# GabeTsai/YOLO-For-Turbines

Measured on AMD Instinct MI355X. Metric: images/sec at 416x416 (fwd), higher is better.
Workload: dtype f32; 1 GPU; BASELINE configs[1]: batch 32/GPU 416x416 fp32 inference, 80-class head, YOLOv3 forward (75 fused conv launches); per_gpu_batch=32, global_batch=32, image_size=416, num_classes=80, parallelism=image-sharded x1 (no collective)

## Files before the change

yolo_for_turbines_amd/csrc/conv_wino4s_f32.hip:

```cpp
#include "split3.h"
#include "wino4_planes.h"
#include "wino4_epilogue.h"

namespace yolo {

struct Wino4SArgs {
    Wino4Args e;
    int nkc;
    int xmap;
};

constexpr int W4S_STAGE = 2 * W4S_PIECE;
constexpr int W4S_SLOTS = 4;
constexpr int W4S_DMA = 3;

template <int OFF>
__device__ __forceinline__ void w4s_read_at(s3_u32x4& f, unsigned addr) {
    asm volatile("ds_read_b128 %0, %1 offset:%2" : "=&v"(f) : "v"(addr), "n"(OFF));
}

template <int ACT, bool RES>
__global__ __launch_bounds__(512, 1) void conv_wino4s_f32(const Wino4SArgs q) {
    extern __shared__ __attribute__((aligned(16))) char smem[];
    const Wino4Args& p = q.e;
    const int tid = threadIdx.x, lane = tid & 63;
    const int wave = __builtin_amdgcn_readfirstlane(tid >> 6);
    const int l16 = lane & 15, kq = lane >> 4;
    const int xcd = blockIdx.x & 7, bq = blockIdx.x >> 3;
    const int row = bq / p.n_nt, wrows = (p.n_whole + 7) >> 3;
    int nt = bq % p.n_nt;
    bool cut = row >= wrows;
    int half = (row - wrows) & 1;
    int mt = cut ? p.n_whole + ((row - wrows) >> 1) * 8 + xcd : row * 8 + xcd;
    if (q.xmap) {
        const int sb = xcd + 8 * (bq >> 5), l = bq & 31, ntg = p.n_mt >> 2;
        cut = true;
        half = l & 1;
        nt = 4 * (sb / ntg) + ((l >> 1) & 3);
        mt = 4 * (sb % ntg) + (l >> 3);
    }
    if (mt >= (cut ? p.n_mt : p.n_whole)) return;
    const int wm = cut ? half : wave & 1, wn = cut ? wave & 3 : wave >> 1;
    const bool busy = !cut || wave < 4;

    int* tab = reinterpret_cast<int*>(smem + W4S_SLOTS * W4S_STAGE);
    wino4_tile_table(p, tab, tid, mt, cut, half);

    const bool dv = cut ? wave >= 4 : wave < 4;
    const int dw = cut ? (wave + 4) & 7 : wave;
    const unsigned own = cut && dv ? (wave - 4) * W4S_PLANE + half * (W4S_PLANE / 2) : 3072 * dw;
    const char* src = (dv ? reinterpret_cast<const char*>(p.V) + (size_t)mt * W4S_PIECE : reinterpret_cast<const char*>(p.U) + (size_t)nt * W4S_PIECE)
                      + (own - (dv ? 0 : W4S_PIECE));
    const size_t s_st = (size_t)(dv ? p.n_mt : p.n_nt) * W4S_PIECE;
    const unsigned lane16 = lane * 16;
    const unsigned lds0 = (unsigned)(size_t)(wn_lptr)smem;
    const unsigned ldsw = lds0 + own;
    const int nkc = q.nkc;
    auto issue_piece = [&](int k, int pass, int g, int slot) {
        const int kc = g / 6, x = g - 6 * kc;
        wn_glds16_s(src + ((size_t)(6 * pass + x) * nkc + kc) * s_st + k * 1024, lane16, ldsw + slot * W4S_STAGE + k * 1024);
    };
    auto issue = [&](int pass, int g, int slot) { wn_for<0, W4S_DMA>([&](auto K) { issue_piece(decltype(K)::value, pass, g, slot); }); };

    const unsigned sw = w4s_slot(l16, kq) * 16;
    const unsigned vb = lds0 + (32 * wm + l16) * 64 + sw;
    const unsigned ub = lds0 + W4S_PIECE + (16 * wn + l16) * 64 + sw;

    f32x4 py[2][4][4];
#pragma unroll
    for (int bb = 0; bb < 2; ++bb)
#pragma unroll
        for (int i = 0; i < 4; ++i)
#pragma unroll
            for (int j = 0; j < 4; ++j) py[bb][i][j] = f32x4{0.f, 0.f, 0.f, 0.f};

    auto run_pass = [&](auto PASS) {
        constexpr int a = decltype(PASS)::value;
        s3_u32x4 uh[2], vh[2][2], um, ul, vm[2], vl[2];
        auto rd_hi = [&](auto SET, unsigned sb) {
            constexpr int S = decltype(SET)::value;
            w4s_read_at<0>(uh[S], ub + sb);
            w4s_read_at<0>(vh[S][0], vb + sb);
            w4s_read_at<1024>(vh[S][1], vb + sb);
        };
        auto rd_vlo = [&](unsigned sb) {
            w4s_read_at<2 * W4S_PLANE>(vl[0], vb + sb);
            w4s_read_at<2 * W4S_PLANE + 1024>(vl[1], vb + sb);
        };
        auto rd_ulo = [&](unsigned sb) { w4s_read_at<2 * W4S_PLANE>(ul, ub + sb); };
        auto rd_vmid = [&](unsigned sb) {
            w4s_read_at<W4S_PLANE>(vm[0], vb + sb);
            w4s_read_at<W4S_PLANE + 1024>(vm[1], vb + sb);
        };
        auto rd_umid = [&](unsigned sb) { w4s_read_at<W4S_PLANE>(um, ub + sb); };
        auto mma = [&](f32x4 (&c)[2], const s3_u32x4& u, const s3_u32x4 (&v)[2]) {
            const s3_bf16x8 fa = __builtin_bit_cast(s3_bf16x8, u);
            c[0] = __builtin_amdgcn_mfma_f32_16x16x32_bf16(fa, __builtin_bit_cast(s3_bf16x8, v[0]), c[0], 0, 0, 0);
            c[1] = __builtin_amdgcn_mfma_f32_16x16x32_bf16(fa, __builtin_bit_cast(s3_bf16x8, v[1]), c[1], 0, 0, 0);
        };
        if constexpr (a == 0) {
            issue(0, 0, 0);
            issue(0, 1, 1);
            issue(0, 2, 2);
        }
        __builtin_amdgcn_sched_barrier(0);
        f32x4 acc[6][2];
#pragma unroll
        for (int x = 0; x < 6; ++x)
#pragma unroll
            for (int bb = 0; bb < 2; ++bb) acc[x][bb] = f32x4{0.f, 0.f, 0.f, 0.f};
#pragma unroll
        for (int x = 0; x < 6; ++x) asm volatile("" : "+v"(acc[x][0]), "+v"(acc[x][1]));
        __builtin_amdgcn_sched_barrier(0);
        wn_wait_vmcnt<2 * W4S_DMA>();
        __builtin_amdgcn_s_barrier();
        __builtin_amdgcn_sched_barrier(0);
        rd_hi(std::integral_constant<int, 0>{}, 0u);
        rd_vlo(0u);
        rd_ulo(0u);
        rd_vmid(0u);
        rd_umid(0u);

        for (int kc = 0; kc < nkc; ++kc) {
            const bool more = kc + 1 < nkc;
            wn_for<0, 6>([&](auto X) {
                constexpr int x = decltype(X)::value, set = x & 1;
                const int g = 6 * kc + x;
                const bool next = x < 5 || more;
                const bool ahead = x < 3 || more;
                const unsigned nb = (unsigned)((g + 1) & (W4S_SLOTS - 1)) * W4S_STAGE;
                const int as = (g + 3) & (W4S_SLOTS - 1);
                __builtin_amdgcn_sched_barrier(0);
                if (next) {
                    if (x < 4 || more) wn_wait_vmcnt<W4S_DMA>();
                    else wn_wait_vmcnt<0>();
                    __builtin_amdgcn_s_barrier();
                }
                __builtin_amdgcn_sched_barrier(0);
                rd_hi(std::integral_constant<int, set ^ 1>{}, nb);
                asm volatile("s_waitcnt lgkmcnt(7)" : "+v"(uh[set]), "+v"(vl[0]), "+v"(vl[1]));
                mma(acc[x], uh[set], vl);
                __builtin_amdgcn_sched_barrier(0);
                if (ahead) issue_piece(0, a, g + 3, as);
                rd_vlo(nb);
                asm volatile("s_waitcnt lgkmcnt(8)" : "+v"(ul), "+v"(vh[set][0]), "+v"(vh[set][1]));
                __builtin_amdgcn_sched_barrier(0);
                mma(acc[x], ul, vh[set]);
                __builtin_amdgcn_sched_barrier(0);
                if (ahead) issue_piece(1, a, g + 3, as);
                rd_ulo(nb);
                asm volatile("s_waitcnt lgkmcnt(6)" : "+v"(um), "+v"(vm[0]), "+v"(vm[1]));
                __builtin_amdgcn_sched_barrier(0);
                mma(acc[x], um, vm);
                __builtin_amdgcn_sched_barrier(0);
                if (ahead) issue_piece(2, a, g + 3, as);
                __builtin_amdgcn_sched_barrier(0);
                mma(acc[x], uh[set], vm);
                __builtin_amdgcn_sched_barrier(0);
                rd_vmid(nb);
                __builtin_amdgcn_sched_barrier(0);
                mma(acc[x], um, vh[set]);
                __builtin_amdgcn_sched_barrier(0);
                rd_umid(nb);
                __builtin_amdgcn_sched_barrier(0);
                mma(acc[x], uh[set], vh[set]);
            });
        }
        asm volatile("s_waitcnt lgkmcnt(0)" ::: "memory");
        __syncthreads();
        if constexpr (a < 5) {
            issue(a + 1, 0, 0);
            issue(a + 1, 1, 1);
            issue(a + 1, 2, 2);
            __builtin_amdgcn_sched_barrier(0);
        }
        wino4_fold_row<a>(acc, py);
    };
    if (busy) {
        run_pass(std::integral_constant<int, 0>{});
        run_pass(std::integral_constant<int, 1>{});
        run_pass(std::integral_constant<int, 2>{});
        run_pass(std::integral_constant<int, 3>{});
        run_pass(std::integral_constant<int, 4>{});
        run_pass(std::integral_constant<int, 5>{});
    } else {
        constexpr int HD = 2;
        const bool mover = wave < 7;
        auto issue_half = [&](int pass, int g, int slot) {
            if (mover) {
                issue_piece(0, pass, g, slot);
                issue_piece(1, pass, g, slot);
            }
        };
        const int ng = 6 * nkc;
        for (int a = 0; a < 6; ++a) {
            if (a == 0) {
                issue_half(0, 0, 0);
                issue_half(0, 1, 1);
                issue_half(0, 2, 2);
            }
            wn_wait_vmcnt<2 * HD>();
            __builtin_amdgcn_s_barrier();
            for (int g = 0; g < ng; ++g) {
                if (g + 1 < ng) {
                    if (g + 2 < ng) wn_wait_vmcnt<HD>();
                    else wn_wait_vmcnt<0>();
                    __builtin_amdgcn_s_barrier();
                }
                if (g + 3 < ng) issue_half(a, g + 3, (g + 3) & (W4S_SLOTS - 1));
            }
            __syncthreads();
            if (a < 5) {
                issue_half(a + 1, 0, 0);
                issue_half(a + 1, 1, 1);
                issue_half(a + 1, 2, 2);
            }
        }
    }

    wino4_epilogue<ACT, RES>(p, smem, tab, py, tid, nt, wm, wn, l16, kq, busy);
}

bool wino4_split_eligible(const yolo_conv_desc* d) {
    if (!wino4_split_supported(d) || d->h != d->w) return false;
    if (d->h == 26 && d->cin == 256 && d->cout == 512) return true;
    if ((d->h == 13 || d->h == 19) && d->cin == 512 && d->cout == 1024) return true;
    return d->h == 52 && d->cin == 128 && d->cout == 256;
}

int conv_wino4s_launch(const yolo_conv_desc* d, const void* x, const float* U4, const void* U_planes, const float* scale, const float* shift,
                       const void* residual, void* y, void* workspace, size_t workspace_bytes, int32_t* nan_flag, hipStream_t s) {
    const Wino4Geom g = wino4_geom(d);
    if (!g.planes) return fail(YOLO_ERR_UNSUPPORTED, "conv winograd F(4x4) on bf16 planes: needs fp32 3x3 stride 1, NHWC output, cin %% 32 == 0");
    const size_t need = g.v_plane_bytes + g.u_plane_bytes;
    if (!workspace || workspace_bytes < need) return fail(YOLO_ERR_WORKSPACE, "conv winograd F(4x4) on bf16 planes: workspace %zu < %zu bytes", workspace_bytes, need);
    if ((size_t)workspace & 15) return fail(YOLO_ERR_ARG, "conv winograd F(4x4) on bf16 planes: workspace must be 16-byte aligned");
    if (!U4 || ((size_t)U4 & 15)) return fail(YOLO_ERR_ARG, "conv winograd F(4x4) on bf16 planes: transformed filters must be 16-byte aligned");
    if ((size_t)U_planes & 15) return fail(YOLO_ERR_ARG, "conv winograd F(4x4) on bf16 planes: filter planes must be 16-byte aligned");
    if (int rc = wino4_planes_launch(g, d, x, U4, U_planes, workspace, s)) return rc;

    Wino4SArgs q;
    Wino4Args& a = q.e;
    a = wino4_gemm_args(g, d, scale, shift, residual, y, nan_flag);
    a.V = (const float*)workspace;
    a.U = (const float*)wino4_u_planes(g, U_planes, workspace);
    q.nkc = g.nkc;
    q.xmap = a.n_whole == 0 && a.n_mt % 4 == 0 && a.n_nt % 4 == 0 && (a.n_mt / 4) * (a.n_nt / 4) % 8 == 0;
    const int grid = q.xmap ? 2 * a.n_mt * a.n_nt : wino4_grid(a);
    const bool res = d->flags & YOLO_FLAG_RESIDUAL;
    const size_t lds = (size_t)W4S_SLOTS * W4S_STAGE + W4_TAB;
    auto go = [&](auto kern) -> int {
        static LdsOnce once;
        if (int rc = reserve_lds(once, reinterpret_cast<const void*>(kern), lds, "conv_wino4s_f32")) return rc;
        hipLaunchKernelGGL(kern, dim3(grid), dim3(512), lds, s, q);
        return check_launch("conv_wino4s_f32");
    };
    YOLO_SWITCH_ACT(d->act, return res ? go(&conv_wino4s_f32<ACT, true>) : go(&conv_wino4s_f32<ACT, false>));
    return fail(YOLO_ERR_ARG, "conv winograd F(4x4) on bf16 planes: activation");
}

}
```

Baseline: 3083 images/s.

## Deepen Winograd split-kernel LDS pipeline to six slots and prefetch across passes

Raises the LDS ring from four to six stage slots so the global-to-LDS loads run five stages ahead instead of three, with each stage's slot fixed by its Winograd index. The prefetch now runs continuously across the six passes, so the next pass's first stages are issued during the tail of the current one. This removes the per-pass __syncthreads and drain/refill bubble. It needs more LDS, which may limit occupancy or the shapes that fit. Per-stage vmcnt waits are rewritten by hand for the final lap, and the epilogue recomputes lane ids with mbcnt.

```diff
diff --git a/yolo_for_turbines_amd/csrc/conv_wino4s_f32.hip b/yolo_for_turbines_amd/csrc/conv_wino4s_f32.hip
--- a/yolo_for_turbines_amd/csrc/conv_wino4s_f32.hip
+++ b/yolo_for_turbines_amd/csrc/conv_wino4s_f32.hip
@@ -11,8 +11,10 @@
 };
 
 constexpr int W4S_STAGE = 2 * W4S_PIECE;
-constexpr int W4S_SLOTS = 4;
+constexpr int W4S_SLOTS = 6;
+constexpr int W4S_AHEAD = W4S_SLOTS - 1;
 constexpr int W4S_DMA = 3;
+static_assert(W4S_SLOTS == 6 && W4S_AHEAD == 5, "the slot of a stage is its xi, and the counted waits of the last lap are written out for five stages ahead");
 
 template <int OFF>
 __device__ __forceinline__ void w4s_read_at(s3_u32x4& f, unsigned addr) {
@@ -56,11 +58,10 @@
     const unsigned lds0 = (unsigned)(size_t)(wn_lptr)smem;
     const unsigned ldsw = lds0 + own;
     const int nkc = q.nkc;
-    auto issue_piece = [&](int k, int pass, int g, int slot) {
-        const int kc = g / 6, x = g - 6 * kc;
-        wn_glds16_s(src + ((size_t)(6 * pass + x) * nkc + kc) * s_st + k * 1024, lane16, ldsw + slot * W4S_STAGE + k * 1024);
+    auto issue_piece = [&](int k, int pass, int kc, int x) {
+        const int xi = kc < nkc ? 6 * pass + x : 6 * pass + 6 + x, c = kc < nkc ? kc : 0;
+        wn_glds16_s(src + ((size_t)xi * nkc + c) * s_st + k * 1024, lane16, ldsw + x * W4S_STAGE + k * 1024);
     };
-    auto issue = [&](int pass, int g, int slot) { wn_for<0, W4S_DMA>([&](auto K) { issue_piece(decltype(K)::value, pass, g, slot); }); };
 
     const unsigned sw = w4s_slot(l16, kq) * 16;
     const unsigned vb = lds0 + (32 * wm + l16) * 64 + sw;
@@ -99,9 +100,7 @@
             c[1] = __builtin_amdgcn_mfma_f32_16x16x32_bf16(fa, __builtin_bit_cast(s3_bf16x8, v[1]), c[1], 0, 0, 0);
         };
         if constexpr (a == 0) {
-            issue(0, 0, 0);
-            issue(0, 1, 1);
-            issue(0, 2, 2);
+            wn_for<0, W4S_AHEAD>([&](auto X) { wn_for<0, W4S_DMA>([&](auto K) { issue_piece(decltype(K)::value, 0, 0, decltype(X)::value); }); });
         }
         __builtin_amdgcn_sched_barrier(0);
         f32x4 acc[6][2];
@@ -112,8 +111,10 @@
 #pragma unroll
         for (int x = 0; x < 6; ++x) asm volatile("" : "+v"(acc[x][0]), "+v"(acc[x][1]));
         __builtin_amdgcn_sched_barrier(0);
-        wn_wait_vmcnt<2 * W4S_DMA>();
-        __builtin_amdgcn_s_barrier();
+        if constexpr (a == 0) {
+            wn_wait_vmcnt<(W4S_AHEAD - 1) * W4S_DMA>();
+            __builtin_amdgcn_s_barrier();
+        }
         __builtin_amdgcn_sched_barrier(0);
         rd_hi(std::integral_constant<int, 0>{}, 0u);
         rd_vlo(0u);
@@ -125,15 +126,18 @@
             const bool more = kc + 1 < nkc;
             wn_for<0, 6>([&](auto X) {
                 constexpr int x = decltype(X)::value, set = x & 1;
-                const int g = 6 * kc + x;
-                const bool next = x < 5 || more;
-                const bool ahead = x < 3 || more;
-                const unsigned nb = (unsigned)((g + 1) & (W4S_SLOTS - 1)) * W4S_STAGE;
-                const int as = (g + 3) & (W4S_SLOTS - 1);
+                const bool on = a < 5 || more;
+                const bool next = x < 5 || on;
+                const bool ahead = x < 1 || on;
+                constexpr int ax = (x + W4S_AHEAD) % W4S_SLOTS;
+                const int akc = x < 1 ? kc : kc + 1;
+                unsigned nb = (unsigned)((x + 1) % W4S_SLOTS) * W4S_STAGE;
+                asm volatile("" : "+s"(nb));
                 __builtin_amdgcn_sched_barrier(0);
                 if (next) {
-                    if (x < 4 || more) wn_wait_vmcnt<W4S_DMA>();
-                    else wn_wait_vmcnt<0>();
+                    constexpr int young = x < 2 ? W4S_AHEAD - 2 : x < 4 ? 4 - x : 0;
+                    if (on) wn_wait_vmcnt<(W4S_AHEAD - 2) * W4S_DMA>();
+                    else wn_wait_vmcnt<young * W4S_DMA>();
                     __builtin_amdgcn_s_barrier();
                 }
                 __builtin_amdgcn_sched_barrier(0);
@@ -141,19 +145,19 @@
                 asm volatile("s_waitcnt lgkmcnt(7)" : "+v"(uh[set]), "+v"(vl[0]), "+v"(vl[1]));
                 mma(acc[x], uh[set], vl);
                 __builtin_amdgcn_sched_barrier(0);
-                if (ahead) issue_piece(0, a, g + 3, as);
+                if (ahead) issue_piece(0, a, akc, ax);
                 rd_vlo(nb);
                 asm volatile("s_waitcnt lgkmcnt(8)" : "+v"(ul), "+v"(vh[set][0]), "+v"(vh[set][1]));
                 __builtin_amdgcn_sched_barrier(0);
                 mma(acc[x], ul, vh[set]);
                 __builtin_amdgcn_sched_barrier(0);
-                if (ahead) issue_piece(1, a, g + 3, as);
+                if (ahead) issue_piece(1, a, akc, ax);
                 rd_ulo(nb);
                 asm volatile("s_waitcnt lgkmcnt(6)" : "+v"(um), "+v"(vm[0]), "+v"(vm[1]));
                 __builtin_amdgcn_sched_barrier(0);
                 mma(acc[x], um, vm);
                 __builtin_amdgcn_sched_barrier(0);
-                if (ahead) issue_piece(2, a, g + 3, as);
+                if (ahead) issue_piece(2, a, akc, ax);
                 __builtin_amdgcn_sched_barrier(0);
                 mma(acc[x], uh[set], vm);
                 __builtin_amdgcn_sched_barrier(0);
@@ -167,13 +171,7 @@
             });
         }
         asm volatile("s_waitcnt lgkmcnt(0)" ::: "memory");
-        __syncthreads();
-        if constexpr (a < 5) {
-            issue(a + 1, 0, 0);
-            issue(a + 1, 1, 1);
-            issue(a + 1, 2, 2);
-            __builtin_amdgcn_sched_barrier(0);
-        }
+        if constexpr (a == 5) __syncthreads();
         wino4_fold_row<a>(acc, py);
     };
     if (busy) {
@@ -186,39 +184,34 @@
     } else {
         constexpr int HD = 2;
         const bool mover = wave < 7;
-        auto issue_half = [&](int pass, int g, int slot) {
+        auto issue_half = [&](int pass, int kc, int x) {
             if (mover) {
-                issue_piece(0, pass, g, slot);
-                issue_piece(1, pass, g, slot);
+                issue_piece(0, pass, kc, x);
+                issue_piece(1, pass, kc, x);
             }
         };
-        const int ng = 6 * nkc;
-        for (int a = 0; a < 6; ++a) {
-            if (a == 0) {
-                issue_half(0, 0, 0);
-                issue_half(0, 1, 1);
-                issue_half(0, 2, 2);
+        for (int x = 0; x < W4S_AHEAD; ++x) issue_half(0, 0, x);
+        wn_wait_vmcnt<(W4S_AHEAD - 1) * HD>();
+        __builtin_amdgcn_s_barrier();
+        for (int a = 0; a < 6; ++a)
+            for (int kc = 0; kc < nkc; ++kc) {
+                const bool on = a < 5 || kc + 1 < nkc;
+                for (int x = 0; x < 6; ++x) {
+                    if (x < 5 || on) {
+                        if (on || x < 2) wn_wait_vmcnt<(W4S_AHEAD - 2) * HD>();
+                        else if (x == 2) wn_wait_vmcnt<2 * HD>();
+                        else if (x == 3) wn_wait_vmcnt<HD>();
+                        else wn_wait_vmcnt<0>();
+                        __builtin_amdgcn_s_barrier();
+                    }
+                    if (x < 1 || on) issue_half(a, x < 1 ? kc : kc + 1, (x + W4S_AHEAD) % W4S_SLOTS);
+                }
             }
-            wn_wait_vmcnt<2 * HD>();
-            __builtin_amdgcn_s_barrier();
-            for (int g = 0; g < ng; ++g) {
-                if (g + 1 < ng) {
-                    if (g + 2 < ng) wn_wait_vmcnt<HD>();
-                    else wn_wait_vmcnt<0>();
-                    __builtin_amdgcn_s_barrier();
-                }
-                if (g + 3 < ng) issue_half(a, g + 3, (g + 3) & (W4S_SLOTS - 1));
-            }
-            __syncthreads();
-            if (a < 5) {
-                issue_half(a + 1, 0, 0);
-                issue_half(a + 1, 1, 1);
-                issue_half(a + 1, 2, 2);
-            }
-        }
+        __syncthreads();
     }
 
-    wino4_epilogue<ACT, RES>(p, smem, tab, py, tid, nt, wm, wn, l16, kq, busy);
+    const int lane_e = __builtin_amdgcn_mbcnt_hi(~0u, __builtin_amdgcn_mbcnt_lo(~0u, 0u));
+    wino4_epilogue<ACT, RES>(p, smem, tab, py, wave * 64 + lane_e, nt, wm, wn, lane_e & 15, lane_e >> 4, busy);
 }
 
 bool wino4_split_eligible(const yolo_conv_desc* d) {
```

Result: faster. 3251 images/s (median of 6 runs) (+5.5%).
